# david-jk/BigGAN-Tensorflow

Hardware: AMD Instinct MI355X
Metric: BigGAN-128 train-step images/sec (higher is better)
Workload: dtype bf16; 1 GPU; BigGAN-128 ch=96 bf16 (BASELINE config 3: global batch 256, 32/GPU over 8 GPUs); img_size=128, ch=96, per_gpu_batch=256, global_batch=256, da_policy=full, g_regularization=ortho_cosine, n_labels=0, gan_type=hinge, hip_graph=False, precision=bf16, parallelism=dp1

## Files before the change

### biggan-tensorflow_amd/csrc/igemm16.hip

```cpp
#include <stdlib.h>

#include "common.h"
#include "igemm.h"
#include "igemm16.h"
#include <type_traits>
#include "igemm_dev.h"

namespace bg {

typedef float f32x4_t __attribute__((ext_vector_type(4)));
typedef float f32x16_t __attribute__((ext_vector_type(16)));
typedef __bf16 bf16x8_t __attribute__((ext_vector_type(8)));
typedef short s16x4v __attribute__((ext_vector_type(4)));
typedef short s16x8v __attribute__((ext_vector_type(8)));
typedef __attribute__((address_space(3))) void lds_void_t;
typedef __attribute__((address_space(1))) const void gbl_void_t;
typedef __attribute__((address_space(3))) s16x4v lds_s16x4v;

__device__ uint4 g_zero_page[1024];

__device__ __forceinline__ void glds16(const void* src, unsigned char* lds_wave_base) {
    __builtin_amdgcn_global_load_lds((gbl_void_t*)src, (lds_void_t*)lds_wave_base, 16, 0, 0);
}

// ... 304 lines not shown
        if (it + 1 < nsteps) stage(cur ^ 1);
        const unsigned char* sbuf = smem + cur * STAGE;
        bf16x8_t a[2][4], b[2][TN];
#pragma unroll
        for (int s2 = 0; s2 < 2; ++s2) {
#pragma unroll
            for (int i = 0; i < 4; ++i)
                a[s2][i] = *reinterpret_cast<const bf16x8_t*>(sbuf + a_row + i * 16 * 128 + koff[s2]);
#pragma unroll
            for (int j = 0; j < TN; ++j)
                b[s2][j] = *reinterpret_cast<const bf16x8_t*>(sbuf + b_row + j * 16 * 128 + koff[s2]);
        }
#pragma unroll
        for (int s2 = 0; s2 < 2; ++s2)
#pragma unroll
            for (int i = 0; i < 4; ++i)
#pragma unroll
                for (int j = 0; j < TN; ++j)
                    acc[i][j] = __builtin_amdgcn_mfma_f32_16x16x32_bf16(b[s2][j], a[s2][i], acc[i][j], 0, 0, 0);
        asm volatile("s_waitcnt vmcnt(0) lgkmcnt(0)" ::: "memory");
        __builtin_amdgcn_s_barrier();
    }

    constexpr int ELD = BN + 4;
    float* est = reinterpret_cast<float*>(smem);
    const bool partial = p.splitk > 1;
    const float alpha = (!partial && p.alpha) ? *p.alpha : 1.0f;
#pragma unroll
    for (int i = 0; i < 4; ++i)
#pragma unroll
        for (int j = 0; j < TN; ++j) {
            const int row = wm * 64 + 16 * i + (lane & 15);
            const int col = wn * 16 * TN + 16 * j + 4 * (lane >> 4);
            f32x4_t v = acc[i][j];
            v[0] *= alpha; v[1] *= alpha; v[2] *= alpha; v[3] *= alpha;
            *reinterpret_cast<f32x4_t*>(est + row * ELD + col) = v;
        }
    __syncthreads();
    constexpr int CPR = BN / 8;
    float* slab = partial ? p.slabs + (int64_t)zs * p.slab_stride : nullptr;
#pragma unroll
    for (int q = 0; q < BM * CPR / 256; ++q) {
        const int idx = t + 256 * q;
        const int row = idx / CPR, cc = idx - row * CPR;
        const int m = m0 + row, col = n0 + cc * 8;
        if (m >= p.M || col >= p.N) continue;
        int64_t ooff;
        if (use_tabo) {
            const unsigned op = tabo[row];
            if (op == 0xffffffffu) continue;
            ooff = (int64_t)op * p.out_ld + col;
        } else if (p.d2s_c) {
            int b, ho, wo;
            if (p.pow2) {
                wo = m & (g.Wo - 1);
                const int t2 = m >> p.wq_shift;
                ho = t2 & (g.Ho - 1);
                b = t2 >> p.hq_shift;
            } else {
                const int t2 = m / g.Wo;
                wo = m - t2 * g.Wo;
                b = t2 / g.Ho;
                ho = t2 - b * g.Ho;
            }
            const int sub = col / p.d2s_c, c = col - sub * p.d2s_c;
            ooff = (((int64_t)b * (2 * g.Ho) + 2 * ho + (sub >> 1)) * (2 * g.Wo) + 2 * wo + (sub & 1)) * p.d2s_c + c;
        } else {
            ooff = (int64_t)m * p.out_ld + col;
        }
        f32x4_t v0 = *reinterpret_cast<const f32x4_t*>(est + row * ELD + cc * 8);
        f32x4_t v1 = *reinterpret_cast<const f32x4_t*>(est + row * ELD + cc * 8 + 4);
        if (partial) {
            *reinterpret_cast<f32x4_t*>(slab + ooff) = v0;
            *reinterpret_cast<f32x4_t*>(slab + ooff + 4) = v1;
            continue;
        }
        if (p.bias) {
            const f32x4_t b0 = *reinterpret_cast<const f32x4_t*>(p.bias + col);
            const f32x4_t b1 = *reinterpret_cast<const f32x4_t*>(p.bias + col + 4);
            v0 += b0;
            v1 += b1;
        }
        if (p.out_f32) {
            float* o = reinterpret_cast<float*>(p.out) + ooff;
            if (p.accumulate) {
                v0 += *reinterpret_cast<const f32x4_t*>(o);
                v1 += *reinterpret_cast<const f32x4_t*>(o + 4);
            }
            *reinterpret_cast<f32x4_t*>(o) = v0;
            *reinterpret_cast<f32x4_t*>(o + 4) = v1;
        } else {
            __bf16* o = reinterpret_cast<__bf16*>(p.out) + ooff;
            if (p.accumulate) {
                const uint4 r = *reinterpret_cast<const uint4*>(o);
                v0[0] += bf16_lo(r.x); v0[1] += bf16_hi(r.x); v0[2] += bf16_lo(r.y); v0[3] += bf16_hi(r.y);
                v1[0] += bf16_lo(r.z); v1[1] += bf16_hi(r.z); v1[2] += bf16_lo(r.w); v1[3] += bf16_hi(r.w);
            }
            uint4 r;
            r.x = pack_bf16x2(v0[0], v0[1]);
            r.y = pack_bf16x2(v0[2], v0[3]);
            r.z = pack_bf16x2(v1[0], v1[1]);
            r.w = pack_bf16x2(v1[2], v1[3]);
            *reinterpret_cast<uint4*>(o) = r;
        }
    }
}

__global__ __launch_bounds__(256) void nn16_slab_reduce_kernel(const float* __restrict__ slabs, void* __restrict__ out,
                                                               const float* __restrict__ bias,
                                                               const float* __restrict__ alpha_dev, int64_t n8, int N,
                                                               int splitk, int64_t slab_stride, int accumulate,
                                                               int out_f32) {
    const float alpha = alpha_dev ? *alpha_dev : 1.0f;
    for (int64_t i = (int64_t)blockIdx.x * 256 + threadIdx.x; i < n8; i += (int64_t)gridDim.x * 256) {
        f32x4_t s0 = {0.f, 0.f, 0.f, 0.f}, s1 = s0;
        for (int z = 0; z < splitk; ++z) {
            const float* sp = slabs + (int64_t)z * slab_stride + i * 8;
            s0 += *reinterpret_cast<const f32x4_t*>(sp);
            s1 += *reinterpret_cast<const f32x4_t*>(sp + 4);
        }
        s0 *= alpha;
        s1 *= alpha;
        if (bias) {
            const int col = (int)((i * 8) % N);
            s0 += *reinterpret_cast<const f32x4_t*>(bias + col);
            s1 += *reinterpret_cast<const f32x4_t*>(bias + col + 4);
        }
        if (out_f32) {
            float* o = reinterpret_cast<float*>(out) + i * 8;
            if (accumulate) {
                s0 += *reinterpret_cast<const f32x4_t*>(o);
                s1 += *reinterpret_cast<const f32x4_t*>(o + 4);
            }
            *reinterpret_cast<f32x4_t*>(o) = s0;
            *reinterpret_cast<f32x4_t*>(o + 4) = s1;
        } else {
            __bf16* o = reinterpret_cast<__bf16*>(out) + i * 8;
            if (accumulate) {
                const uint4 r = *reinterpret_cast<const uint4*>(o);
                s0[0] += bf16_lo(r.x); s0[1] += bf16_hi(r.x); s0[2] += bf16_lo(r.y); s0[3] += bf16_hi(r.y);
                s1[0] += bf16_lo(r.z); s1[1] += bf16_hi(r.z); s1[2] += bf16_lo(r.w); s1[3] += bf16_hi(r.w);
            }
            uint4 r;
            r.x = pack_bf16x2(s0[0], s0[1]);
            r.y = pack_bf16x2(s0[2], s0[3]);
            r.z = pack_bf16x2(s1[0], s1[1]);
            r.w = pack_bf16x2(s1[2], s1[3]);
            *reinterpret_cast<uint4*>(o) = r;
        }
    }
}

constexpr int NH_T = 16;
template <int NT> struct NHGeom {
    static constexpr int HW = NH_T + NT - 1;
    static constexpr int NPIX = HW * HW;
    static constexpr int A_INSTR = (NPIX * 8 + 511) / 512;
    static constexpr int A_BYTES = A_INSTR * 8192;
};
constexpr int nh_w_instr(int NF) { return (32 * NF * 8 + 511) / 512; }
constexpr int NH_WS = 2;
template <int NT, int NF> constexpr int nn16h_lds_bytes() {
    const int ring = NHGeom<NT>::A_BYTES + NH_WS * nh_w_instr(NF) * 8192;
    const int epi = 128 * (32 * NF + 4) * 4;
    return ring > epi ? ring : epi;
}

struct NHTile {
    int b, y0, x0, n0, ph, pw, phase, nph, tx, ty, tiles_x, tiles_y;
};
template <int NF, int THIN>
__device__ __forceinline__ void nn16h_epilogue(const NN16Params& p, const NHTile& tl, f32x4_t (&acc)[4][NF],
                                               unsigned char* smem) {
    constexpr int BN = 32 * NF;
    const Gather& g = p.g;
    const int t = threadIdx.x, lane = t & 63, w = t >> 6;
    const int wm = w >> 1, wn = w & 1;
    const int px = lane & 15, kb = lane >> 4;
    const int b = tl.b, y0 = tl.y0, x0 = tl.x0, n0 = tl.n0, ph = tl.ph, pw = tl.pw, phase = tl.phase, nph = tl.nph;
    const int tx = tl.tx, ty = tl.ty, tiles_x = tl.tiles_x, tiles_y = tl.tiles_y;
    constexpr int ELD = BN + 4;
    float* est = reinterpret_cast<float*>(smem);
    const float alpha = p.alpha ? *p.alpha : 1.0f;
    constexpr int CPR = BN / 8;
    constexpr int RG = 512 / BN;
    for (int half = 0; half < 2; ++half) {
        if ((wm >> 1) == half) {
#pragma unroll
            for (int i = 0; i < 4; ++i)
#pragma unroll
                for (int j = 0; j < NF; ++j) {
                    const int row = ((wm & 1) * 4 + i) * 16 + px;
                    const int col = wn * 16 * NF + 16 * j + 4 * kb;
                    f32x4_t v = acc[i][j];
                    v[0] *= alpha; v[1] *= alpha; v[2] *= alpha; v[3] *= alpha;
                    *reinterpret_cast<f32x4_t*>(est + row * ELD + col) = v;
                }
        }
        __syncthreads();
        for (int idx = t; idx < 128 * CPR; idx += 512) {
            const int row = idx / CPR, cc = idx - row * CPR;
            const int gy = y0 + 8 * half + (row >> 4), gx = x0 + (row & 15);
            const int col = THIN == 1 ? 0 : n0 + cc * 8;
            const int oy = THIN == 1 ? 2 * gy + (cc >> 1) : gy * g.pstep + ph;
            const int ox = THIN == 1 ? 2 * gx + (cc & 1) : gx * g.pstep + pw;
            f32x4_t v0 = *reinterpret_cast<const f32x4_t*>(est + row * ELD + cc * 8);
            f32x4_t v1 = *reinterpret_cast<const f32x4_t*>(est + row * ELD + cc * 8 + 4);
            const bool live = gy < g.Hq && gx < g.Wq && col < p.N && oy < g.Ho && ox < g.Wo;
            if (live) {
                int64_t ooff = ((int64_t)(b * g.Ho + oy) * g.Wo + ox) * p.out_ld + col;
                if (THIN == 0 && p.d2s_c) {
                    const int sub = col / p.d2s_c, c = col - sub * p.d2s_c;
                    ooff = (((int64_t)b * (2 * g.Ho) + 2 * oy + (sub >> 1)) * (2 * g.Wo) + 2 * ox + (sub & 1)) * p.d2s_c + c;
                }
                if (p.bias) {
                    v0 += *reinterpret_cast<const f32x4_t*>(p.bias + col);
                    v1 += *reinterpret_cast<const f32x4_t*>(p.bias + col + 4);
                }
                if (p.out_f32) {
                    float* o = reinterpret_cast<float*>(p.out) + ooff;
                    if (p.accumulate) {
                        v0 += *reinterpret_cast<const f32x4_t*>(o);
                        v1 += *reinterpret_cast<const f32x4_t*>(o + 4);
                    }
                    *reinterpret_cast<f32x4_t*>(o) = v0;
                    *reinterpret_cast<f32x4_t*>(o + 4) = v1;
                } else {
                    __bf16* o = reinterpret_cast<__bf16*>(p.out) + ooff;
                    if (p.accumulate) {
                        const uint4 rr = *reinterpret_cast<const uint4*>(o);
                        v0[0] += bf16_lo(rr.x); v0[1] += bf16_hi(rr.x); v0[2] += bf16_lo(rr.y); v0[3] += bf16_hi(rr.y);
                        v1[0] += bf16_lo(rr.z); v1[1] += bf16_hi(rr.z); v1[2] += bf16_lo(rr.w); v1[3] += bf16_hi(rr.w);
                    }
                    uint4 rr;
                    rr.x = pack_bf16x2(v0[0], v0[1]);
                    rr.y = pack_bf16x2(v0[2], v0[3]);
                    rr.z = pack_bf16x2(v1[0], v1[1]);
                    rr.w = pack_bf16x2(v1[2], v1[3]);
                    *reinterpret_cast<uint4*>(o) = rr;
                    if (p.stats_part) {
                        v0[0] = bf16_lo(rr.x); v0[1] = bf16_hi(rr.x); v0[2] = bf16_lo(rr.y); v0[3] = bf16_hi(rr.y);
                        v1[0] = bf16_lo(rr.z); v1[1] = bf16_hi(rr.z); v1[2] = bf16_lo(rr.w); v1[3] = bf16_hi(rr.w);
                    }
                }
            } else if (p.stats_part) {
                v0 = f32x4_t{0.f, 0.f, 0.f, 0.f};
                v1 = v0;
            }
            if (p.stats_part) {
                *reinterpret_cast<f32x4_t*>(est + row * ELD + cc * 8) = v0;
                *reinterpret_cast<f32x4_t*>(est + row * ELD + cc * 8 + 4) = v1;
            }
        }
        __syncthreads();
        if (p.stats_part) {
            float st_s = 0.f, st_q = 0.f;
            if (t < RG * BN) {
                const int colr = t % BN;
                for (int row = t / BN; row < 128; row += RG) {
                    const float v = est[row * ELD + colr];
                    st_s += v;
                    st_q = fmaf(v, v, st_q);
                }
            }
            __syncthreads();
            if (t < RG * BN) {
                est[t] = st_s;
                est[RG * BN + t] = st_q;
            }
            __syncthreads();
            if (t < BN && n0 + t < p.N) {
                float s = 0.f, q = 0.f;
#pragma unroll
                for (int r2 = 0; r2 < RG; ++r2) {
                    s += est[r2 * BN + t];
                    q += est[RG * BN + r2 * BN + t];
                }
                const int64_t prow = 2 * ((((int64_t)b * tiles_y + ty) * tiles_x + tx) * nph + phase) + half;
                p.stats_part[prow * (2 * (int64_t)p.N) + n0 + t] = s;
                p.stats_part[prow * (2 * (int64_t)p.N) + p.N + n0 + t] = q;
            }
            __syncthreads();
        }
    }
}

template <int NT, int NF, int MODE, int THIN = 0>
__global__ __launch_bounds__(512, 4) void nn16h_kernel(const NN16Params p) {
    using G = NHGeom<NT>;
    constexpr int WW = G::HW, NPIX = G::NPIX, A_INSTR = G::A_INSTR, A_BYTES = G::A_BYTES;
    constexpr int BN = 32 * NF, W_INSTR = nh_w_instr(NF), W_BYTES = W_INSTR * 8192, NTAPS = NT * NT;
    extern __shared__ __attribute__((aligned(16))) unsigned char smem[];

    const int t = threadIdx.x, lane = t & 63, w = t >> 6;
    const int wm = w >> 1, wn = w & 1;
    const Gather& g = p.g;

    const int nph = g.pstep * g.pstep;
    const int tiles_x = (g.Wq + NH_T - 1) / NH_T, tiles_y = (g.Hq + NH_T - 1) / NH_T;
    const int nt = (p.N + BN - 1) / BN;
    int r = xcd_remap(blockIdx.x, gridDim.x);
    int phase, tile_n, tx, ty, b;
    if (p.mfast) {
        tx = r % tiles_x; r /= tiles_x;
        ty = r % tiles_y; r /= tiles_y;
        b = r % g.Nb; r /= g.Nb;
        phase = r % nph;
        tile_n = r / nph;
    } else {
        phase = r % nph; r /= nph;
        tile_n = r % nt; r /= nt;
        tx = r % tiles_x; r /= tiles_x;
        ty = r % tiles_y;
        b = r / tiles_y;
    }
    const int y0 = ty * NH_T, x0 = tx * NH_T, n0 = tile_n * BN;
    int ph = 0, pw = 0;
    if (MODE == GATHER_TCONV && g.pstep > 1) {
        ph = g.pstep - 1 - phase / g.pstep;
        pw = g.pstep - 1 - phase % g.pstep;
    }
    int base_h, base_w, kh0 = 0, kw0 = 0, kstep = 1;
    if (MODE == GATHER_CONV) {
        base_h = base_w = -g.pad;
    } else if (g.pstep > 1) {
        kstep = g.stride;
        kh0 = (ph + g.pad) % g.stride;
        kw0 = (pw + g.pad) % g.stride;
        base_h = (ph + g.pad - kh0) / g.stride - (NT - 1);
        base_w = (pw + g.pad - kw0) / g.stride - (NT - 1);
    } else {
        base_h = base_w = g.pad - (NT - 1);
    }
    int nkh = NT, nkw = NT;
    if (MODE == GATHER_TCONV && NT == 2 && g.pstep > 1) {
        nkh = (g.k - kh0 + kstep - 1) / kstep;
        nkw = (g.k - kw0 + kstep - 1) / kstep;
    }
    const int ntaps = (MODE == GATHER_TCONV && NT == 2) ? nkh * nkw : NTAPS;

    const unsigned char* abase = reinterpret_cast<const unsigned char*>(p.A);
    const unsigned char* bbase = reinterpret_cast<const unsigned char*>(p.B);
    const unsigned char* zero = reinterpret_cast<const unsigned char*>(g_zero_page);
    const uint32_t lds0 = static_cast<uint32_t>(
        reinterpret_cast<uintptr_t>((__attribute__((address_space(3))) unsigned char*)smem));
    const uint32_t ldsw = lds0 + A_BYTES;

    const unsigned char* asrc[A_INSTR];
    int acb[A_INSTR];
#pragma unroll
    for (int i = 0; i < A_INSTR; ++i) {
        const int pp = (i * 8 + w) * 64 + lane;
        const int q = pp >> 3, c = (pp & 7) ^ (q & 6);
        const int hy = q / WW, hx = q - hy * WW;
        int sy = y0 + hy + base_h, sx = x0 + hx + base_w;
        bool ok = q < NPIX;
        if (MODE == GATHER_CONV && g.reflect) {
            sy = sy < 0 ? -sy : sy;
            sy = sy >= g.Hs ? 2 * (g.Hs - 1) - sy : sy;
            sx = sx < 0 ? -sx : sx;
            sx = sx >= g.Ws ? 2 * (g.Ws - 1) - sx : sx;
        }
        ok = ok && sy >= 0 && sy < g.Hs && sx >= 0 && sx < g.Ws;
        acb[i] = 16 * c;
        asrc[i] = ok ? abase + 2 * ((int64_t)((b * g.Hs + sy) * g.Ws + sx) * g.ld) : zero;
    }
    const unsigned char* wsrc[W_INSTR];
    int wcb[W_INSTR];
    bool wok[W_INSTR];
    int wrow[W_INSTR];
#pragma unroll
    for (int i = 0; i < W_INSTR; ++i) {
        const int pp = (i * 8 + w) * 64 + lane;
        const int n = pp >> 3, c = (pp & 7) ^ ((n >> 1) & 7);
        wok[i] = n < BN && n0 + n < p.N;
        wcb[i] = 16 * c;
        wrow[i] = n;
        wsrc[i] = bbase + 2 * ((int64_t)(THIN == 1 ? (n & 7) : n0 + n) * p.C);
    }
    const uint32_t dma_a = __builtin_amdgcn_readfirstlane(lds0 + w * 1024);
    const uint32_t dma_w = __builtin_amdgcn_readfirstlane(ldsw + w * 1024);

    auto issue_a = [&](int chunk) {
        const uint32_t dst = dma_a;
        const int cb = chunk * 128;
#pragma unroll
        for (int i = 0; i < A_INSTR; ++i) {
            const bool cv = (cb + acb[i]) < 2 * p.C;
            glds16_asm(cv ? asrc[i] + (cb + acb[i]) : zero, dst + i * 8192);
        }
    };
    auto issue_w = [&](int step) {
        const int chunk = step / ntaps, tap = step - chunk * ntaps;
        const int ty_ = tap / nkw;
        const int hy = NT - nkh + ty_, hx = NT - nkw + (tap - ty_ * nkw);
        const int kh = MODE == GATHER_CONV ? hy : kh0 + kstep * (NT - 1 - hy);
        const int kw = MODE == GATHER_CONV ? hx : kw0 + kstep * (NT - 1 - hx);
        const int64_t toff = 2 * ((int64_t)(kh * g.k + kw) * p.tap_stride);
        const uint32_t dst = dma_w + (step % NH_WS) * W_BYTES;
        const int cb = chunk * 128;
#pragma unroll
        for (int i = 0; i < W_INSTR; ++i) {
            bool cv = wok[i] && (cb + wcb[i]) < 2 * p.C;
            int64_t to = toff;
            if (THIN == 1) {
                const int kty = ((wrow[i] >> 4) & 1) + 1 - 2 * hy, ktx = ((wrow[i] >> 3) & 1) + 1 - 2 * hx;
                cv = cv && kty >= 0 && ktx >= 0;
                to = 2 * ((int64_t)(kty * 3 + ktx) * p.tap_stride);
            }
            glds16_asm(cv ? wsrc[i] + to + (cb + wcb[i]) : zero, dst + i * 8192);
        }
    };

    const int px = lane & 15, kb = lane >> 4;
    int qb[4];
#pragma unroll
    for (int i = 0; i < 4; ++i) qb[i] = (wm * 4 + i) * WW + px;
    uint32_t boff[NF];
#pragma unroll
    for (int j = 0; j < NF; ++j) {
        const int n = wn * 16 * NF + 16 * j + px;
        boff[j] = A_BYTES + n * 128 + 16 * (kb ^ ((n >> 1) & 7));
    }

    f32x4_t acc[4][NF];
#pragma unroll
    for (int i = 0; i < 4; ++i)
#pragma unroll
        for (int j = 0; j < NF; ++j)
#pragma unroll
            for (int e = 0; e < 4; ++e) acc[i][j][e] = 0.f;

    const int nchunks = (p.C + 63) >> 6;
    const int T = nchunks * ntaps;
    issue_a(0);
    issue_w(0);

    for (int step = 0; step < T; ++step) {
        const int chunk = step / ntaps, tap = step - chunk * ntaps;
        asm volatile("s_waitcnt vmcnt(0) lgkmcnt(0)" ::: "memory");
        __builtin_amdgcn_s_barrier();
        if (step + 1 < T) {
            if (tap == ntaps - 1) {
            } else {
                issue_w(step + 1);
            }
        }

        const int ty_ = tap / nkw;
        const int hy = NT - nkh + ty_, hx = NT - nkw + (tap - ty_ * nkw);
        const uint32_t abuf = 0;
        const uint32_t wslot = (uint32_t)(step % NH_WS) * W_BYTES;
        const int tq = hy * WW + hx;
        const int ksteps = (p.C - chunk * 64) >= 64 ? 2 : 1;
        uint32_t aaddr[4];
#pragma unroll
        for (int i = 0; i < 4; ++i) {
            const int q = qb[i] + tq;
            aaddr[i] = abuf + q * 128 + 16 * (kb ^ (q & 6));
        }
#pragma unroll
        for (int s2 = 0; s2 < 2; ++s2) {
            if (s2 < ksteps) {
                bf16x8_t a[4], bw[NF];
#pragma unroll
                for (int i = 0; i < 4; ++i)
                    a[i] = *reinterpret_cast<const bf16x8_t*>(smem + (aaddr[i] ^ (s2 ? 64u : 0u)));
#pragma unroll
                for (int j = 0; j < NF; ++j)
                    bw[j] = *reinterpret_cast<const bf16x8_t*>(smem + ((boff[j] + wslot) ^ (s2 ? 64u : 0u)));
#pragma unroll
                for (int i = 0; i < 4; ++i)
#pragma unroll
                    for (int j = 0; j < NF; ++j)
                        acc[i][j] = __builtin_amdgcn_mfma_f32_16x16x32_bf16(bw[j], a[i], acc[i][j], 0, 0, 0);
            }
        }
        if (tap == ntaps - 1 && step + 1 < T) {
            asm volatile("s_waitcnt lgkmcnt(0)" ::: "memory");
            __builtin_amdgcn_s_barrier();
            issue_a(chunk + 1);
            issue_w(step + 1);
        }
    }
    asm volatile("s_waitcnt vmcnt(0) lgkmcnt(0)" ::: "memory");
    __builtin_amdgcn_s_barrier();

    NHTile tl;
    tl.b = b; tl.y0 = y0; tl.x0 = x0; tl.n0 = n0; tl.ph = ph; tl.pw = pw; tl.phase = phase; tl.nph = nph;
    tl.tx = tx; tl.ty = ty; tl.tiles_x = tiles_x; tl.tiles_y = tiles_y;
    nn16h_epilogue<NF, THIN>(p, tl, acc, smem);
}

constexpr int TN16_BK = 64;
constexpr int TN16_TILE = TN16_BK * 256;

__device__ __forceinline__ s16x4v lds_tr16(uint32_t lds_byte_addr) {
    return __builtin_amdgcn_ds_read_tr16_b64_v4i16(reinterpret_cast<lds_s16x4v*>(lds_byte_addr));
}
__device__ __forceinline__ int tr16_swz(int row, int chunk) {
    return 256 * row + 16 * (chunk ^ (((row & 3) << 2) | ((row >> 2) & 3)));
}

template <int MODE>
__global__ __launch_bounds__(256, 2) void tn16_kernel(const TN16Params p) {
    constexpr int BM = 128, BN = 128;
    extern __shared__ __attribute__((aligned(16))) unsigned char smem[];

    const int t = threadIdx.x;
    const int lane = t & 63, w = t >> 6;
    const int wm = w >> 1, wn = w & 1;
    const Gather& g = p.g;

    const int ntile = p.tiles_m * p.tiles_n;
    const int lin = xcd_remap(blockIdx.x, ntile * p.splitk);
    const int zs = lin / ntile;
    const int tile = lin - zs * ntile;
    const int tile_n = tile % p.tiles_n, tile_m = tile / p.tiles_n;
    const int mf0 = tile_m * BM, cb0 = tile_n * BN;
    const int row_begin = zs * p.rows_per_split;
    const int row_end = min(p.M, row_begin + p.rows_per_split);
    const int nsteps = max(0, (row_end - row_begin + TN16_BK - 1) / TN16_BK);

    const int prow = lane >> 4;
    const int ch = (lane & 15) ^ ((prow << 2) | w);
    const int mf = mf0 + 8 * ch;
    int a_kh = 0, a_kw = 0, a_c = mf;
    if (MODE != GATHER_PLAIN) {
        const int tap = mf / p.Ca;
        a_c = mf - tap * p.Ca;
        a_kh = tap / g.k;
        a_kw = tap - a_kh * g.k;
    }
    const bool a_ok = mf < p.Mf;
    const int cb = cb0 + 8 * ch;
    const bool b_ok = cb < p.Cb;
    const __bf16* Ab = reinterpret_cast<const __bf16*>(p.A);
    const __bf16* Bb = reinterpret_cast<const __bf16*>(p.Bv);
    const void* zero = reinterpret_cast<const void*>(g_zero_page);
    int m_next = row_begin + 4 * w + prow;

    auto stage = [&](int buf) {
        unsigned char* sa = smem + buf * (2 * TN16_TILE) + (4 * w) * 256;
        unsigned char* sb = sa + TN16_TILE;
#pragma unroll
        for (int j = 0; j < 4; ++j) {
            const int m = m_next + 16 * j;
            const void* srca = zero;
            const void* srcb = zero;
            if (m < row_end) {
                if (a_ok) {
                    int64_t pix;
                    if (MODE == GATHER_PLAIN) {
                        pix = m;
                    } else {
                        int b, ho, wo;
                        if (p.pow2) {
                            wo = m & (g.Wq - 1);
                            const int r = m >> p.wq_shift;
                            ho = r & (g.Hq - 1);
                            b = r >> p.hq_shift;
                        } else {
                            wo = m % g.Wq;
                            const int r = m / g.Wq;
                            ho = r % g.Hq;
                            b = r / g.Hq;
                        }
                        const int hs = conv_src(ho, a_kh, g.stride, g.pad, g.reflect, g.Hs);
                        const int ws = conv_src(wo, a_kw, g.stride, g.pad, g.reflect, g.Ws);
                        pix = (hs >= 0 && ws >= 0) ? ((int64_t)b * g.Hs + hs) * g.Ws + ws : -1;
                    }
                    if (pix >= 0) srca = Ab + pix * g.ld + a_c;
                }
                if (b_ok) srcb = Bb + (int64_t)m * p.b_ld + cb;
            }
            glds16(srca, sa + j * 16 * 256);
            glds16(srcb, sb + j * 16 * 256);
        }
        m_next += TN16_BK;
    };

    f32x16_t acc[2][2];
#pragma unroll
    for (int i = 0; i < 2; ++i)
#pragma unroll
        for (int j = 0; j < 2; ++j)
#pragma unroll
            for (int r = 0; r < 16; ++r) acc[i][j][r] = 0.f;

    const int kblk = lane >> 5, g16 = (lane >> 4) & 1, q = (lane & 15) >> 2, pq = lane & 3;
    const uint32_t lds0 = static_cast<uint32_t>(
        reinterpret_cast<uintptr_t>((__attribute__((address_space(3))) unsigned char*)smem));
    uint32_t a_ad[2][2], b_ad[2][2];
#pragma unroll
    for (int jj = 0; jj < 2; ++jj) {
        const int row = 8 * kblk + 4 * jj + q;
#pragma unroll
        for (int i = 0; i < 2; ++i) {
            a_ad[i][jj] = lds0 + tr16_swz(row, 4 * (wm * 2 + i) + 2 * g16 + (pq >> 1)) + 8 * (pq & 1);
            b_ad[i][jj] = lds0 + TN16_TILE + tr16_swz(row, 4 * (wn * 2 + i) + 2 * g16 + (pq >> 1)) + 8 * (pq & 1);
        }
    }
    auto operand = [&](uint32_t lo_addr, uint32_t hi_addr) {
        const s16x4v lo = lds_tr16(lo_addr), hi = lds_tr16(hi_addr);
        const s16x8v v = __builtin_shufflevector(lo, hi, 0, 1, 2, 3, 4, 5, 6, 7);
        return __builtin_bit_cast(bf16x8_t, v);
    };

    if (nsteps > 0) stage(0);
    __syncthreads();
    for (int it = 0; it < nsteps; ++it) {
        const int cur = it & 1;
        if (it + 1 < nsteps) stage(cur ^ 1);
        const uint32_t bufoff = (uint32_t)cur * (2u * TN16_TILE);
#pragma unroll
        for (int s = 0; s < TN16_BK / 16; ++s) {
            bf16x8_t a[2], b[2];
#pragma unroll
            for (int i = 0; i < 2; ++i) a[i] = operand(a_ad[i][0] + bufoff + 4096 * s, a_ad[i][1] + bufoff + 4096 * s);
#pragma unroll
            for (int j = 0; j < 2; ++j) b[j] = operand(b_ad[j][0] + bufoff + 4096 * s, b_ad[j][1] + bufoff + 4096 * s);
#pragma unroll
            for (int i = 0; i < 2; ++i)
#pragma unroll
                for (int j = 0; j < 2; ++j)
                    acc[i][j] = __builtin_amdgcn_mfma_f32_32x32x16_bf16(a[i], b[j], acc[i][j], 0, 0, 0);
        }
        __syncthreads();
    }

    float* obase = p.out + (int64_t)zs * p.slab_stride;
#pragma unroll
    for (int i = 0; i < 2; ++i) {
#pragma unroll
        for (int r = 0; r < 16; ++r) {
            const int row = mf0 + wm * 64 + 32 * i + (r & 3) + 8 * (r >> 2) + 4 * (lane >> 5);
// ... 262 lines not shown
        int k0 = 0, kstep = 1, nk = g.k;
        if (mode == GATHER_TCONV && g.pstep > 1) {
            kstep = g.stride;
            k0 = (ph + g.pad) % g.stride;
            nk = (g.k - k0 + g.stride - 1) / g.stride;
        }
        for (int q = 0; q < nq; ++q) {
            const int o = q * g.pstep + ph;
            for (int i = 0; i < nk; ++i) {
                const int kk = k0 + i * kstep;
                bool ok;
                if (mode == GATHER_CONV) {
                    const int src = o * g.stride + kk - g.pad;
                    ok = g.reflect || (src >= 0 && src < n_src);
                } else {
                    const int hn = o + g.pad - kk;
                    ok = hn >= 0 && hn % g.stride == 0 && hn / g.stride < n_src;
                }
                valid += ok;
            }
            slots += nk;
        }
    }
    return slots ? (double)valid / (double)slots : 1.0;
}

static double nn16_posmajor_fraction(const NN16Params& p, int mode) {
    const char* e = getenv("BG_NN16_POSMAJOR");
    if (e && atoi(e) == 0) return 1.0;
    const Gather& g = p.g;
    if (g.k <= 1 || g.Nb < 16 || g.Hq <= 0 || g.Wq <= 0 || (int64_t)g.Hq * g.Wq > 40 * 40) return 1.0;
    const double f = nn16_axis_fraction(g, mode, g.Hq, g.Hs) * nn16_axis_fraction(g, mode, g.Wq, g.Ws);
    return f < 0.9 ? f : 1.0;
}

static NN16Plan plan_nn16(const NN16Params& p, int mode, int zdim, bool allow_split) {
    static const int slots = getenv("BG_NN16_SLOTS") ? atoi(getenv("BG_NN16_SLOTS")) : 512;
    const int64_t tm = (p.M + NN16_BM - 1) / NN16_BM;
    int steps = nn16_steps_min(p, mode);
    const double pm = nn16_posmajor_fraction(p, mode);
    if (pm < 1.0) steps = max(1, (int)(steps * pm + 0.5));
    NN16Plan best{4, 1};
    double best_cost = 1e30;
    for (int tn = 4; tn >= 1; --tn) {
        const int bn = 32 * tn;
        const int64_t tiles = tm * ((p.N + bn - 1) / bn) * zdim;
        const double unit = 1.5 + tn;
        const int max_sk = allow_split ? (steps / 4 < 16 ? (steps / 4 < 1 ? 1 : steps / 4) : 16) : 1;
        for (int sk = 1; sk <= max_sk; ++sk) {
            const int64_t rounds = (tiles * sk + slots - 1) / slots;
            double cost = (double)rounds * ((steps + sk - 1) / sk + 2.0) * unit;
            if (sk > 1) cost += 6.0 * unit + 0.02 * sk * (double)tiles / slots * bn;
            if (cost < best_cost - 1e-9) {
                best_cost = cost;
                best = NN16Plan{tn, sk};
            }
        }
    }
    return best;
}

size_t nn16_workspace_bytes(const NN16Params& p, int mode, int zdim, int64_t out_elems) {
    const NN16Plan pl = plan_nn16(p, mode, zdim, true);
    return pl.splitk > 1 ? (size_t)pl.splitk * out_elems * sizeof(float) : 0;
}

static int nn16_mfast(const NN16Params& p, int tiles_m, int tiles_n);

template <int TN>
static int launch_nn16_ring_inst(const NN16Params& p, dim3 grid, hipStream_t s) {
    constexpr int lds = nn16_lds_bytes(TN, NN16_RING_TAPS);
    if (!lds_opt_in(reinterpret_cast<const void*>(&nn16_kernel<TN, GATHER_TCONV, true, true>), lds)) return BG_ERR_LAUNCH;
    hipLaunchKernelGGL((nn16_kernel<TN, GATHER_TCONV, true, true>), grid, dim3(256), lds, s, p);
    return BG_OK;
}

int launch_nn16_ring(NN16Params& p, hipStream_t s) {
    BG_REQUIRE(p.ring == 1 && (p.ring_lines == 1 || p.ring_lines == 2), "nn16 ring launch: ring = 1, ring_lines 1 or 2");
    BG_REQUIRE(p.g.k >= 1 && p.g.k <= NN16_RING_TAPS / 2 && p.g.Ho >= 4 && p.g.Wo >= 4 && p.accumulate == 1,
               "nn16 ring launch: kernel size %d / map %d x %d not supported", p.g.k, p.g.Ho, p.g.Wo);
    BG_REQUIRE(p.C % 8 == 0 && p.N % 8 == 0 && p.g.ld % 8 == 0 && p.out_ld % 8 == 0, "nn16 ring launch: channels %% 8");
    const int npos = p.ring_lines * p.g.Wo + p.ring_lines * (p.g.Ho - p.ring_lines);
    p.g.pstep = 1;
    p.g.Hq = 1;
    p.g.Wq = npos;
    p.M = p.g.Nb * npos;
    p.posmajor = 1;
    p.splitk = 1;
    p.slabs = nullptr;
    p.zfold = 0;
    p.pow2 = 0;
    int tn = 4, best = 1 << 30;
    for (int c = 4; c >= 1; --c) {
        const int padded = (p.N + 32 * c - 1) / (32 * c) * (32 * c);
        if (padded < best) { best = padded; tn = c; }
    }
    p.tiles_m = (p.M + NN16_BM - 1) / NN16_BM;
    p.tiles_n = (p.N + 32 * tn - 1) / (32 * tn);
    p.mfast = nn16_mfast(p, p.tiles_m, p.tiles_n);
    dim3 grid(p.tiles_m * p.tiles_n, 1, 1);
    int rc;
    switch (tn) {
        case 1: rc = launch_nn16_ring_inst<1>(p, grid, s); break;
        case 2: rc = launch_nn16_ring_inst<2>(p, grid, s); break;
        case 3: rc = launch_nn16_ring_inst<3>(p, grid, s); break;
        default: rc = launch_nn16_ring_inst<4>(p, grid, s); break;
    }
    if (rc) return rc;
    BG_LAUNCH_CHECK();
    return BG_OK;
}

template <int TN, int MODE, bool PM>
static int launch_nn16_inst(const NN16Params& p, dim3 grid, hipStream_t s) {
    constexpr int lds = nn16_lds_bytes(TN);
    if (!lds_opt_in(reinterpret_cast<const void*>(&nn16_kernel<TN, MODE, PM>), lds)) return BG_ERR_LAUNCH;
    prof_kernel("nn16_kernel<%d, %d, %s>", TN, MODE, PM ? "true" : "false");
    hipLaunchKernelGGL((nn16_kernel<TN, MODE, PM>), grid, dim3(256), lds, s, p);
    return BG_OK;
}

template <int MODE, bool PM>
static int launch_nn16_pm(const NN16Params& p, int tn, dim3 grid, hipStream_t s) {
    switch (tn) {
        case 1: return launch_nn16_inst<1, MODE, PM>(p, grid, s);
        case 2: return launch_nn16_inst<2, MODE, PM>(p, grid, s);
        case 3: return launch_nn16_inst<3, MODE, PM>(p, grid, s);
        default: return launch_nn16_inst<4, MODE, PM>(p, grid, s);
    }
}

template <int MODE>
static int launch_nn16_mode(const NN16Params& p, int tn, dim3 grid, hipStream_t s) {
    return p.posmajor ? launch_nn16_pm<MODE, true>(p, tn, grid, s) : launch_nn16_pm<MODE, false>(p, tn, grid, s);
}

static int nn16h_taps(const NN16Params& p, int mode, int zdim) {
    const char* e = getenv("BG_NN16_HALO");
    const int use = e ? atoi(e) : 1;
    static const int cmax = getenv("BG_NN16_HALO_CMAX") ? atoi(getenv("BG_NN16_HALO_CMAX")) : 4096;
    const Gather& g = p.g;
    if (!use || p.C > cmax || p.C % 32 || p.N % 8 || g.Hq < NH_T || g.Wq < NH_T || g.Hq % NH_T || g.Wq % NH_T) return 0;
    if (mode == GATHER_CONV) return (g.stride == 1 && g.k == 3 && g.pstep == 1 && zdim == 1) ? 3 : 0;
    if (g.reflect) return 0;
    if (g.stride == 1 && g.k == 3 && g.pstep == 1 && zdim == 1) return 3;
    if (g.stride == 2 && g.k == 4 && g.pstep == 2 && zdim == 4) return 2;
    if (g.stride == 2 && g.k == 3 && g.pad == 1 && g.pstep == 2 && zdim == 4) {
        const char* e3 = getenv("BG_NN16_HALO_K3S2");
        return (e3 && atoi(e3) == 1) ? 2 : 0;
    }
    return 0;
}

template <int NT, int NF, int MODE>
static int launch_nn16h_inst(const NN16Params& p, int blocks, hipStream_t s) {
    constexpr int lds = nn16h_lds_bytes<NT, NF>();
    if (!lds_opt_in(reinterpret_cast<const void*>(&nn16h_kernel<NT, NF, MODE>), lds)) return BG_ERR_LAUNCH;
    prof_kernel("nn16h_kernel<%d, %d, %d>", NT, NF, MODE);
    hipLaunchKernelGGL((nn16h_kernel<NT, NF, MODE>), dim3(blocks), dim3(512), lds, s, p);
    return BG_OK;
}

template <int NT, int MODE>
static int launch_nn16h_nf(const NN16Params& p, int nf, int blocks, hipStream_t s) {
    switch (nf) {
        case 1: return launch_nn16h_inst<NT, 1, MODE>(p, blocks, s);
        case 2: return launch_nn16h_inst<NT, 2, MODE>(p, blocks, s);
        case 3: return launch_nn16h_inst<NT, 3, MODE>(p, blocks, s);
        default: return launch_nn16h_inst<NT, 4, MODE>(p, blocks, s);
    }
}

bool nn16h_d2s_ok(const NN16Params& p) {
    const char* e = getenv("BG_THIN_D2S");
    const int use = e ? atoi(e) : 1;
    const Gather& g = p.g;
    return use && p.N == 8 && p.out_ld == 8 && g.k == 3 && g.stride == 2 && g.pad == 1 && !g.reflect && p.C % 32 == 0 &&
           g.Hs % NH_T == 0 && g.Ws % NH_T == 0 && g.Ho == 2 * g.Hs && g.Wo == 2 * g.Ws && !p.bias && !p.stats_part;
}
int launch_nn16h_d2s(const NN16Params& plain, hipStream_t s) {
    BG_REQUIRE(nn16h_d2s_ok(plain), "nn16h depth-to-space form: unsupported geometry");
    NN16Params p = plain;
    Gather& g = p.g;
    g.Hq = g.Hs; g.Wq = g.Ws; g.pstep = 1; g.pad = 0; g.stride = 1;
    p.N = 32;
    p.splitk = 1; p.mfast = 0; p.ring = 0;
    const int64_t blocks = (int64_t)g.Nb * (g.Hq / NH_T) * (g.Wq / NH_T);
    BG_REQUIRE(blocks > 0 && blocks < (int64_t(1) << 31), "nn16h: grid out of range");
    constexpr int lds = nn16h_lds_bytes<2, 1>();
    if (!lds_opt_in(reinterpret_cast<const void*>(&nn16h_kernel<2, 1, GATHER_CONV, 1>), lds)) return BG_ERR_LAUNCH;
    prof_kernel("nn16h_kernel<2, 1, 0, d2s>");
    hipLaunchKernelGGL((nn16h_kernel<2, 1, GATHER_CONV, 1>), dim3((int)blocks), dim3(512), lds, s, p);
    BG_LAUNCH_CHECK();
    return BG_OK;
}

static int nn16_mfast(const NN16Params& p, int tiles_m, int tiles_n) {
    const char* e = getenv("BG_NN16_MFAST");
    if (!e) return 0;
    if (strcmp(e, "auto") != 0) return atoi(e) != 0;
    const double l2 = 3.0e6;
    const double a_bytes = 2.0 * p.g.Nb * (double)p.g.Hs * p.g.Ws * p.g.ld;
    const double w_bytes = 2.0 * p.g.k * p.g.k * (double)p.N * p.C;
    const double nfast = a_bytes + (w_bytes > l2 ? w_bytes * tiles_m : w_bytes);
    const double mfast = w_bytes + (a_bytes > l2 ? a_bytes * tiles_n : a_bytes);
    return mfast < nfast;
}

static int launch_nn16h(NN16Params& p, int mode, int ntaps, hipStream_t s) {
    int nf = 4, best = 1 << 30;
    for (int c = 4; c >= 1; --c) {
        const int padded = (p.N + 32 * c - 1) / (32 * c) * (32 * c);
        if (padded < best) { best = padded; nf = c; }
    }
    const Gather& g = p.g;
    const int64_t blocks = (int64_t)g.Nb * (g.Hq / NH_T) * (g.Wq / NH_T) * ((p.N + 32 * nf - 1) / (32 * nf)) *
                           (g.pstep * g.pstep);
    BG_REQUIRE(blocks > 0 && blocks < (int64_t(1) << 31), "nn16h: grid out of range");
    p.splitk = 1;
    p.mfast = nn16_mfast(p, g.Nb * (g.Hq / NH_T) * (g.Wq / NH_T), (p.N + 32 * nf - 1) / (32 * nf));
    int rc;
    if (mode == GATHER_CONV) rc = launch_nn16h_nf<3, GATHER_CONV>(p, nf, (int)blocks, s);
    else if (ntaps == 3) rc = launch_nn16h_nf<3, GATHER_TCONV>(p, nf, (int)blocks, s);
    else rc = launch_nn16h_nf<2, GATHER_TCONV>(p, nf, (int)blocks, s);
    if (rc) return rc;
    BG_LAUNCH_CHECK();
    return BG_OK;
}

bool nn16_d2s_ok(const NN16Params& p, int mode, int zdim) {
    const Gather& g = p.g;
    if (p.d2s_c <= 0 || p.d2s_c % 8 || p.N != 4 * p.d2s_c || p.C % 8 || mode != GATHER_CONV || zdim != 1 || g.stride != 1 ||
        g.pstep != 1 || g.Hq != g.Ho || g.Wq != g.Wo || p.stats_part || p.ring)
        return false;
    if ((int64_t)g.Nb * g.Ho * g.Wo * 4 >= (int64_t(1) << 31)) return false;
    if (nn16h_taps(p, mode, zdim)) return true;
    if (nn16_posmajor_fraction(p, mode) < 1.0) return false;
    return plan_nn16(p, mode, zdim, true).splitk == 1;
}

int64_t nn16_stats_rows(const NN16Params& p, int mode, int zdim) {
    if (p.C % 8 || p.N % 8 || !nn16h_taps(p, mode, zdim)) return 0;
    return 2 * (int64_t)p.g.Nb * (p.g.Hq / NH_T) * (p.g.Wq / NH_T) * (p.g.pstep * p.g.pstep);
}

int launch_nn16(NN16Params& p, int mode, int zdim, int64_t out_elems, void* ws, size_t ws_bytes, hipStream_t s) {
    BG_REQUIRE(p.C % 8 == 0 && p.N % 8 == 0 && p.g.ld % 8 == 0 && p.out_ld % 8 == 0,
               "bf16-resident conv: channel counts must be multiples of 8 (C=%d N=%d)", p.C, p.N);
    BG_REQUIRE((reinterpret_cast<uintptr_t>(p.A) & 15) == 0 && (reinterpret_cast<uintptr_t>(p.B) & 15) == 0 &&
                   (reinterpret_cast<uintptr_t>(p.out) & 15) == 0,
               "bf16-resident conv: tensors must be 16-byte aligned");
    BG_REQUIRE(p.g.k >= 1 && p.g.k <= NN16_TAPS && p.C <= 8192 && p.g.stride >= 1 && p.g.stride <= 2,
               "bf16-resident conv: kernel size %d / stride %d / %d channels not supported", p.g.k, p.g.stride, p.C);
    BG_REQUIRE((int64_t)p.g.Nb * p.g.Hs * p.g.Ws < (int64_t(1) << 30) && (int64_t)p.g.Nb * p.g.Ho * p.g.Wo < (int64_t(1) << 31),
               "bf16-resident conv: more than 2^30 source / 2^31 output pixels");
    BG_REQUIRE(p.d2s_c == 0 || (nn16_d2s_ok(p, mode, zdim) && ws == nullptr),
               "bf16-resident conv: this launch has no depth-to-space store (bg_conv2d_fwd_d2s_supported)");
    if (const int ntaps = nn16h_taps(p, mode, zdim)) return launch_nn16h(p, mode, ntaps, s);
    BG_REQUIRE(p.stats_part == nullptr, "bf16-resident conv: fused statistics need the halo-tile form (nn16_stats_rows)");
    NN16Plan pl = plan_nn16(p, mode, zdim, ws != nullptr);
    if (pl.splitk > 1 && ws_bytes < (size_t)pl.splitk * out_elems * sizeof(float)) pl.splitk = 1;
    p.splitk = pl.splitk;
    p.slabs = reinterpret_cast<float*>(ws);
    p.slab_stride = out_elems;
    const int bn = 32 * pl.tn;
    p.tiles_m = (p.M + NN16_BM - 1) / NN16_BM;
    p.tiles_n = (p.N + bn - 1) / bn;
    p.pow2 = 0;
    if (p.g.Wq > 0 && p.g.Hq > 0 && (p.g.Wq & (p.g.Wq - 1)) == 0 && (p.g.Hq & (p.g.Hq - 1)) == 0) {
        p.pow2 = 1;
        p.wq_shift = __builtin_ctz(p.g.Wq);
        p.hq_shift = __builtin_ctz(p.g.Hq);
    }
    p.posmajor = nn16_posmajor_fraction(p, mode) < 1.0;
    p.mfast = nn16_mfast(p, p.tiles_m, p.tiles_n);
    dim3 grid(p.tiles_m * p.tiles_n, 1, zdim * p.splitk);
    p.zfold = 0;
    if (mode == GATHER_TCONV && zdim > 1 && p.splitk == 1 && p.g.k % p.g.stride == 0) {
        p.zfold = zdim;
        grid = dim3(p.tiles_m * p.tiles_n * zdim, 1, 1);
    }
    int rc;
    if (mode == GATHER_CONV)
        rc = launch_nn16_mode<GATHER_CONV>(p, pl.tn, grid, s);
    else
        rc = launch_nn16_mode<GATHER_TCONV>(p, pl.tn, grid, s);
    if (rc) return rc;
    BG_LAUNCH_CHECK();
    if (pl.splitk > 1) {
        const int64_t n8 = out_elems / 8;
        int blocks = (int)((n8 + 255) / 256);
        if (blocks > 2048) blocks = 2048;
        hipLaunchKernelGGL(nn16_slab_reduce_kernel, dim3(blocks), dim3(256), 0, s, p.slabs, p.out, p.bias, p.alpha, n8,
                           p.N, pl.splitk, out_elems, p.accumulate, p.out_f32);
        BG_LAUNCH_CHECK();
    }
    return BG_OK;
}

static void plan_tn16(TN16Params& p) {
    const int64_t tiles = (int64_t)((p.Mf + 127) / 128) * ((p.Cb + 127) / 128);
    static const int want = getenv("BG_TN16_WANT") ? atoi(getenv("BG_TN16_WANT")) : 1024;
    int sk = (int)(want / tiles);
    const int max_sk = (p.M + 4 * TN16_BK - 1) / (4 * TN16_BK);
    if (sk > max_sk) sk = max_sk;
    if (sk < 1) sk = 1;
    if (sk > 512) sk = 512;
    int rps = (p.M + sk - 1) / sk;
    rps = (rps + TN16_BK - 1) / TN16_BK * TN16_BK;
    p.splitk = (p.M + rps - 1) / rps;
    p.rows_per_split = rps;
}

static int tn16x_nbi(const TN16Params& p) {
    const char* e = getenv("BG_TN16X_NBI");
    if (!e || atoi(e) != 2) return 1;
    return (p.Cb >= 512 && p.Cb % 256 == 0 && p.Mf >= 256) ? 2 : 1;
}

static bool plan_tn16x(const TN16Params& p, int* sk_out, int* rps_out) {
    static const int use_wide = getenv("BG_TN16_WIDE") ? atoi(getenv("BG_TN16_WIDE")) : 1;
    if (!use_wide || p.Mf <= 128 || p.M < 8 * TN16_BK) return false;
    if (p.g.k > 0 && (p.g.Wq <= 0 || p.g.Hq <= 0 || (p.g.Wq & (p.g.Wq - 1)) || (p.g.Hq & (p.g.Hq - 1)))) return false;
    const int nbi = tn16x_nbi(p);
    const int tm = (p.Mf + 255) / 256, tn = (p.Cb + 128 * nbi - 1) / (128 * nbi);
    static const int wantx0 = getenv("BG_TN16X_WANT") ? atoi(getenv("BG_TN16X_WANT")) : 512;
    const int wantx = nbi == 2 ? wantx0 / 2 : wantx0;
    int sk = wantx / (tm * tn);
    const int max_sk = (p.M + 4 * TN16_BK - 1) / (4 * TN16_BK);
    if (sk > max_sk) sk = max_sk;
    if (sk < 1) sk = 1;
    if (sk > 512) sk = 512;
    int rps = (p.M + sk - 1) / sk;
    rps = (rps + TN16_BK - 1) / TN16_BK * TN16_BK;
    *sk_out = (p.M + rps - 1) / rps;
    *rps_out = rps;
    return true;
}

size_t tn16_workspace_bytes(const TN16Params& p0) {
    TN16Params p = p0;
    plan_tn16(p);
    int sk = p.splitk, skx = 1, rps = 0;
    if (plan_tn16x(p0, &skx, &rps) && skx > sk) sk = skx;
    return sk > 1 ? (size_t)sk * p.Mf * p.Cb * sizeof(float) : 0;
// ... 101 lines not shown
```

Measured before the change: 2611 images/sec.

## Shrink halo-conv LDS ring to 1KB rounds and unroll step loop by slot

Sizes the halo implicit-GEMM kernel's LDS ring by 1 KB wave rounds instead of whole 8 KB instructions, skipping the surplus DMA issues, so the LDS footprint shrinks and the static_assert targets two blocks per CU. Per-lane swizzle offsets become single scalars instead of per-instruction arrays, which cuts register use. The step loop is unrolled by weight slot with compile-time slot offsets and incremental tap/chunk counters, replacing per-step divisions. This risks layout mismatches in the reworked swizzle formula and adds code complexity.

```diff
diff --git a/biggan-tensorflow_amd/csrc/igemm16.hip b/biggan-tensorflow_amd/csrc/igemm16.hip
--- a/biggan-tensorflow_amd/csrc/igemm16.hip
+++ b/biggan-tensorflow_amd/csrc/igemm16.hip
@@ -480,16 +480,19 @@
 }
 
 constexpr int NH_T = 16;
+constexpr int NH_LDS_MAX = 81920;
 template <int NT> struct NHGeom {
     static constexpr int HW = NH_T + NT - 1;
     static constexpr int NPIX = HW * HW;
-    static constexpr int A_INSTR = (NPIX * 8 + 511) / 512;
-    static constexpr int A_BYTES = A_INSTR * 8192;
+    static constexpr int A_ROUNDS = (NPIX * 8 + 63) / 64;
+    static constexpr int A_INSTR = (A_ROUNDS + 7) / 8;
+    static constexpr int A_BYTES = A_ROUNDS * 1024;
 };
-constexpr int nh_w_instr(int NF) { return (32 * NF * 8 + 511) / 512; }
+constexpr int nh_w_rounds(int NF) { return 32 * NF * 8 / 64; }
+constexpr int nh_w_instr(int NF) { return (nh_w_rounds(NF) + 7) / 8; }
 constexpr int NH_WS = 2;
 template <int NT, int NF> constexpr int nn16h_lds_bytes() {
-    const int ring = NHGeom<NT>::A_BYTES + NH_WS * nh_w_instr(NF) * 8192;
+    const int ring = NHGeom<NT>::A_BYTES + NH_WS * nh_w_rounds(NF) * 1024;
     const int epi = 128 * (32 * NF + 4) * 4;
     return ring > epi ? ring : epi;
 }
@@ -616,11 +619,17 @@
 template <int NT, int NF, int MODE, int THIN = 0>
 __global__ __launch_bounds__(512, 4) void nn16h_kernel(const NN16Params p) {
     using G = NHGeom<NT>;
-    constexpr int WW = G::HW, NPIX = G::NPIX, A_INSTR = G::A_INSTR, A_BYTES = G::A_BYTES;
-    constexpr int BN = 32 * NF, W_INSTR = nh_w_instr(NF), W_BYTES = W_INSTR * 8192, NTAPS = NT * NT;
+    constexpr int WW = G::HW, NPIX = G::NPIX, A_ROUNDS = G::A_ROUNDS, A_INSTR = G::A_INSTR, A_BYTES = G::A_BYTES;
+    constexpr int BN = 32 * NF, W_ROUNDS = nh_w_rounds(NF), W_INSTR = nh_w_instr(NF), W_BYTES = W_ROUNDS * 1024;
+    constexpr int NTAPS = NT * NT;
+    static_assert(NH_WS == 2, "the step loop below alternates between two slots");
+    static_assert(nn16h_lds_bytes<NT, NF>() <= NH_LDS_MAX, "two blocks per CU");
+    static_assert(128 * (BN + 4) * 4 <= nn16h_lds_bytes<NT, NF>(), "the epilogue's staging tile overlays the ring");
+    static_assert(A_BYTES % 1024 == 0 && W_BYTES % 1024 == 0, "every LDS-DMA destination is 1 KB aligned");
     extern __shared__ __attribute__((aligned(16))) unsigned char smem[];
 
     const int t = threadIdx.x, lane = t & 63, w = t >> 6;
+    const int wu = __builtin_amdgcn_readfirstlane(w);
     const int wm = w >> 1, wn = w & 1;
     const Gather& g = p.g;
 
@@ -674,12 +683,12 @@
         reinterpret_cast<uintptr_t>((__attribute__((address_space(3))) unsigned char*)smem));
     const uint32_t ldsw = lds0 + A_BYTES;
 
+    const int acb = 16 * ((lane & 7) ^ ((lane >> 3) & 6));
     const unsigned char* asrc[A_INSTR];
-    int acb[A_INSTR];
 #pragma unroll
     for (int i = 0; i < A_INSTR; ++i) {
         const int pp = (i * 8 + w) * 64 + lane;
-        const int q = pp >> 3, c = (pp & 7) ^ (q & 6);
+        const int q = pp >> 3;
         const int hy = q / WW, hx = q - hy * WW;
         int sy = y0 + hy + base_h, sx = x0 + hx + base_w;
         bool ok = q < NPIX;
@@ -690,19 +699,17 @@
             sx = sx >= g.Ws ? 2 * (g.Ws - 1) - sx : sx;
         }
         ok = ok && sy >= 0 && sy < g.Hs && sx >= 0 && sx < g.Ws;
-        acb[i] = 16 * c;
         asrc[i] = ok ? abase + 2 * ((int64_t)((b * g.Hs + sy) * g.Ws + sx) * g.ld) : zero;
     }
+    const int wcb = 16 * ((lane & 7) ^ (4 * (w & 1) + (lane >> 4)));
     const unsigned char* wsrc[W_INSTR];
-    int wcb[W_INSTR];
     bool wok[W_INSTR];
     int wrow[W_INSTR];
 #pragma unroll
     for (int i = 0; i < W_INSTR; ++i) {
         const int pp = (i * 8 + w) * 64 + lane;
-        const int n = pp >> 3, c = (pp & 7) ^ ((n >> 1) & 7);
+        const int n = pp >> 3;
         wok[i] = n < BN && n0 + n < p.N;
-        wcb[i] = 16 * c;
         wrow[i] = n;
         wsrc[i] = bbase + 2 * ((int64_t)(THIN == 1 ? (n & 7) : n0 + n) * p.C);
     }
@@ -712,31 +719,31 @@
     auto issue_a = [&](int chunk) {
         const uint32_t dst = dma_a;
         const int cb = chunk * 128;
+        const bool cv = (cb + acb) < 2 * p.C;
 #pragma unroll
         for (int i = 0; i < A_INSTR; ++i) {
-            const bool cv = (cb + acb[i]) < 2 * p.C;
-            glds16_asm(cv ? asrc[i] + (cb + acb[i]) : zero, dst + i * 8192);
+            if (8 * (i + 1) > A_ROUNDS && 8 * i + wu >= A_ROUNDS) continue;
+            glds16_asm(cv ? asrc[i] + (cb + acb) : zero, dst + i * 8192);
         }
     };
-    auto issue_w = [&](int step) {
-        const int chunk = step / ntaps, tap = step - chunk * ntaps;
-        const int ty_ = tap / nkw;
-        const int hy = NT - nkh + ty_, hx = NT - nkw + (tap - ty_ * nkw);
+    auto issue_w = [&](int chunk, int ty_, int tx_, int slot) {
+        const int hy = NT - nkh + ty_, hx = NT - nkw + tx_;
         const int kh = MODE == GATHER_CONV ? hy : kh0 + kstep * (NT - 1 - hy);
         const int kw = MODE == GATHER_CONV ? hx : kw0 + kstep * (NT - 1 - hx);
         const int64_t toff = 2 * ((int64_t)(kh * g.k + kw) * p.tap_stride);
-        const uint32_t dst = dma_w + (step % NH_WS) * W_BYTES;
+        const uint32_t dst = dma_w + slot * W_BYTES;
         const int cb = chunk * 128;
 #pragma unroll
         for (int i = 0; i < W_INSTR; ++i) {
-            bool cv = wok[i] && (cb + wcb[i]) < 2 * p.C;
+            if (8 * (i + 1) > W_ROUNDS && 8 * i + wu >= W_ROUNDS) continue;
+            bool cv = wok[i] && (cb + wcb) < 2 * p.C;
             int64_t to = toff;
             if (THIN == 1) {
                 const int kty = ((wrow[i] >> 4) & 1) + 1 - 2 * hy, ktx = ((wrow[i] >> 3) & 1) + 1 - 2 * hx;
                 cv = cv && kty >= 0 && ktx >= 0;
                 to = 2 * ((int64_t)(kty * 3 + ktx) * p.tap_stride);
             }
-            glds16_asm(cv ? wsrc[i] + to + (cb + wcb[i]) : zero, dst + i * 8192);
+            glds16_asm(cv ? wsrc[i] + to + (cb + wcb) : zero, dst + i * 8192);
         }
     };
 
@@ -761,31 +768,41 @@
 
     const int nchunks = (p.C + 63) >> 6;
     const int T = nchunks * ntaps;
+    int c_chunk = 0, c_ty = 0, c_tx = 0;
+    int w_chunk = 0, w_ty = 0, w_tx = 0, w_step = 0;
+    auto issue_next_w = [&](int slot) {
+        if (w_step < T) {
+            issue_w(w_chunk, w_ty, w_tx, slot);
+            ++w_step;
+            if (++w_tx == nkw) {
+                w_tx = 0;
+                if (++w_ty == nkh) {
+                    w_ty = 0;
+                    ++w_chunk;
+                }
+            }
+        }
+    };
+    issue_next_w(0);
     issue_a(0);
-    issue_w(0);
-
-    for (int step = 0; step < T; ++step) {
-        const int chunk = step / ntaps, tap = step - chunk * ntaps;
+
+    auto hstep = [&](int step, auto slot_c) {
+        constexpr int SLOT = decltype(slot_c)::value;
+        constexpr int NEXT = SLOT ^ 1;
         asm volatile("s_waitcnt vmcnt(0) lgkmcnt(0)" ::: "memory");
         __builtin_amdgcn_s_barrier();
-        if (step + 1 < T) {
-            if (tap == ntaps - 1) {
-            } else {
-                issue_w(step + 1);
-            }
-        }
-
-        const int ty_ = tap / nkw;
-        const int hy = NT - nkh + ty_, hx = NT - nkw + (tap - ty_ * nkw);
-        const uint32_t abuf = 0;
-        const uint32_t wslot = (uint32_t)(step % NH_WS) * W_BYTES;
+        const bool reload = c_ty == nkh - 1 && c_tx == nkw - 1 && step + 1 < T;
+        if (!reload) issue_next_w(NEXT);
+
+        const int hy = NT - nkh + c_ty, hx = NT - nkw + c_tx;
+        constexpr uint32_t wslot = (uint32_t)SLOT * W_BYTES;
         const int tq = hy * WW + hx;
-        const int ksteps = (p.C - chunk * 64) >= 64 ? 2 : 1;
+        const int ksteps = (p.C - c_chunk * 64) >= 64 ? 2 : 1;
         uint32_t aaddr[4];
 #pragma unroll
         for (int i = 0; i < 4; ++i) {
             const int q = qb[i] + tq;
-            aaddr[i] = abuf + q * 128 + 16 * (kb ^ (q & 6));
+            aaddr[i] = q * 128 + 16 * (kb ^ (q & 6));
         }
 #pragma unroll
         for (int s2 = 0; s2 < 2; ++s2) {
@@ -796,7 +813,7 @@
                     a[i] = *reinterpret_cast<const bf16x8_t*>(smem + (aaddr[i] ^ (s2 ? 64u : 0u)));
 #pragma unroll
                 for (int j = 0; j < NF; ++j)
-                    bw[j] = *reinterpret_cast<const bf16x8_t*>(smem + ((boff[j] + wslot) ^ (s2 ? 64u : 0u)));
+                    bw[j] = *reinterpret_cast<const bf16x8_t*>(smem + ((boff[j] ^ (s2 ? 64u : 0u)) + wslot));
 #pragma unroll
                 for (int i = 0; i < 4; ++i)
 #pragma unroll
@@ -804,12 +821,23 @@
                         acc[i][j] = __builtin_amdgcn_mfma_f32_16x16x32_bf16(bw[j], a[i], acc[i][j], 0, 0, 0);
             }
         }
-        if (tap == ntaps - 1 && step + 1 < T) {
+        if (reload) {
             asm volatile("s_waitcnt lgkmcnt(0)" ::: "memory");
             __builtin_amdgcn_s_barrier();
-            issue_a(chunk + 1);
-            issue_w(step + 1);
-        }
+            issue_a(c_chunk + 1);
+            issue_next_w(NEXT);
+        }
+        if (++c_tx == nkw) {
+            c_tx = 0;
+            if (++c_ty == nkh) {
+                c_ty = 0;
+                ++c_chunk;
+            }
+        }
+    };
+    for (int step = 0; step < T; step += NH_WS) {
+        hstep(step, std::integral_constant<int, 0>());
+        if (step + 1 < T) hstep(step + 1, std::integral_constant<int, 1>());
     }
     asm volatile("s_waitcnt vmcnt(0) lgkmcnt(0)" ::: "memory");
     __builtin_amdgcn_s_barrier();
@@ -1378,12 +1406,13 @@
     return 0;
 }
 
-template <int NT, int NF, int MODE>
+template <int NT, int NF, int MODE, int THIN = 0>
 static int launch_nn16h_inst(const NN16Params& p, int blocks, hipStream_t s) {
     constexpr int lds = nn16h_lds_bytes<NT, NF>();
-    if (!lds_opt_in(reinterpret_cast<const void*>(&nn16h_kernel<NT, NF, MODE>), lds)) return BG_ERR_LAUNCH;
-    prof_kernel("nn16h_kernel<%d, %d, %d>", NT, NF, MODE);
-    hipLaunchKernelGGL((nn16h_kernel<NT, NF, MODE>), dim3(blocks), dim3(512), lds, s, p);
+    if (!lds_opt_in(reinterpret_cast<const void*>(&nn16h_kernel<NT, NF, MODE, THIN>), lds)) return BG_ERR_LAUNCH;
+    if (THIN) prof_kernel("nn16h_kernel<%d, %d, %d, d2s>", NT, NF, MODE);
+    else prof_kernel("nn16h_kernel<%d, %d, %d>", NT, NF, MODE);
+    hipLaunchKernelGGL((nn16h_kernel<NT, NF, MODE, THIN>), dim3(blocks), dim3(512), lds, s, p);
     return BG_OK;
 }
 
@@ -1413,10 +1442,7 @@
     p.splitk = 1; p.mfast = 0; p.ring = 0;
     const int64_t blocks = (int64_t)g.Nb * (g.Hq / NH_T) * (g.Wq / NH_T);
     BG_REQUIRE(blocks > 0 && blocks < (int64_t(1) << 31), "nn16h: grid out of range");
-    constexpr int lds = nn16h_lds_bytes<2, 1>();
-    if (!lds_opt_in(reinterpret_cast<const void*>(&nn16h_kernel<2, 1, GATHER_CONV, 1>), lds)) return BG_ERR_LAUNCH;
-    prof_kernel("nn16h_kernel<2, 1, 0, d2s>");
-    hipLaunchKernelGGL((nn16h_kernel<2, 1, GATHER_CONV, 1>), dim3((int)blocks), dim3(512), lds, s, p);
+    if (const int rc = launch_nn16h_inst<2, 1, GATHER_CONV, 1>(p, (int)blocks, s)) return rc;
     BG_LAUNCH_CHECK();
     return BG_OK;
 }
```

Result: faster. 2665 images/sec (median of 6 runs) (+2.1%).
